# alv-around/mini-stark

Measured on AMD Instinct MI355X. Metric: stark_proofs_per_s, higher is better.
Workload: dtype u64; 1 GPU; Fibonacci AIR, Goldilocks, 2^20 trace rows, blowup 8, 20 security bits (w=3, c=6, rounds=23, ood_queries=1, fri_queries=2); a step = 8 independent proofs in flight per GPU

## Files before the change

### mini-stark_amd/csrc/ctx.hpp

```cpp
#pragma once
#include "../../include/ministark.h"

#include <cstdarg>
#include <cstdio>
#include <cstdlib>
#include <map>
#include <new>
#include <string>
#include <type_traits>
#include <vector>

#include "field.hpp"
#include "merkle.hpp"
#include "ntt.hpp"
#include "poly.hpp"

namespace msctx {

struct DevBuf {
  void* p = nullptr; size_t cap = 0;
  int ensure(size_t bytes) {
    if (bytes <= cap) return 0;
    if (p) msrt::free_dev(p);
    p = nullptr; cap = 0;
// ... 154 lines not shown
  msrt::HostFlag arm_flag() { if (!poll_sync || prof_on) return msrt::HostFlag{nullptr, 0}; seq_pending = ++seq_no; return msrt::HostFlag{host_seq(), seq_pending}; }
  void launched() { seq_armed = seq_pending; seq_pending = 0; }
  bool arm_next_eval = false;
  const unsigned long long* fwd_next_eval = nullptr;
  unsigned long long* host_aux2() const { return host_seq() + 1; }
  unsigned long long* validity_len_dev = nullptr; bool validity_len_host = false; size_t validity_ncoef = 0;
  DevBuf d_evdone;
  int ensure_evdone() { if (!d_evdone.p) { if (d_evdone.ensure(256)) return fail(MS_ERR_NOMEM, "length word"); CK(msrt::memset_dev(d_evdone.p, 0, 256, stream)); } return 0; }
  int sync_results() { const unsigned long long a = seq_armed; seq_armed = 0; return a ? msrt::sync_flag(stream, host_seq(), a) : msrt::sync(stream); }
  template <class K> int run_coop(int kid, unsigned gx, int threads, size_t lds, const typename K::Params& p, unsigned gy = 1) {
    launched();
    if (gx == 0 || gy == 0) return 0;
    if (!prof_on) return msrt::launch_coop<K>(stream, gx, gy, threads, lds, p);
    ProfRec r; r.kid = kid; r.sub = next_sub; r.bytes = next_bytes; r.part = part_depth > 0; next_bytes = 0; next_sub = 0;
    if (msrt::event_create(&r.a) || msrt::event_create(&r.b)) return 1;
    msrt::event_record(r.a, stream);
    int e = msrt::launch_coop<K>(stream, gx, gy, threads, lds, p);
    msrt::event_record(r.b, stream);
    prof_recs.push_back(r);
    return e;
  }
  template <class K> int run(int kid, unsigned gx, unsigned gy, int threads, size_t lds, const typename K::Params& p) {
    launched();
    if (gx == 0 || gy == 0) return 0;
    if (!prof_on) return msrt::launch<K>(stream, gx, gy, threads, lds, p);
    ProfRec r; r.kid = kid; r.sub = next_sub; r.bytes = next_bytes; r.part = part_depth > 0; next_bytes = 0; next_sub = 0;
    if (msrt::event_create(&r.a) || msrt::event_create(&r.b)) return 1;
    msrt::event_record(r.a, stream);
    int e = msrt::launch<K>(stream, gx, gy, threads, lds, p);
    msrt::event_record(r.b, stream);
    prof_recs.push_back(r);
    return e;
  }
  int profile_begin() override { prof_on = true; return 0; }
  int profile_end(char* out, size_t cap) override;

  struct Plan {
    int log_n = 0, log_r0 = 0, log_rho = 0, npass = 0, K[4] = {0, 0, 0, 0}, lo_bits = 0;
    int LC[4] = {msntt::TILE_LOG_C, msntt::TILE_LOG_C, msntt::TILE_LOG_C, msntt::TILE_LOG_C};
    bool v2[4] = {false, false, false, false};
    bool regp[4] = {false, false, false, false};
    DevBuf tw_lo, tw_hi, w_r[4], vtw, w0;
    T n_inv = 0;
  };
  std::map<int, Plan*> plans;
  DevBuf ntt_scratch;
  int ntt_kmax = 9;
  int ntt_v2 = 1, ntt_v2_regpass = 1;
  int ntt_fast = 1;

  int get_plan(int log_n, int log_pad, bool inverse, Plan** out);

  template <bool INV, int K, int TH>
  int launch_fast(const msntt::PassParams<F>& pp, size_t tiles, size_t batch);
  template <class KK> int launch_v2i(const msntt::PassParams<F>& pp, unsigned grid, int nsub, int mode, int k, int lc);
  template <bool INV, int K, int LC, int MODE>
  int launch_v2m(const msntt::PassParams<F>& pp, size_t tiles, size_t batch);
  int ntt_coop_wgs = 512, ntt_share = 1;
  unsigned coop_grid(size_t work_items, int per_cu = 2) const { const size_t g = (size_t)ntt_coop_wgs * per_cu / 2; return (unsigned)(work_items < g ? work_items : g); }
  template <bool INV, int K, int LC>
  int launch_v2(const msntt::PassParams<F>& pp, size_t tiles, size_t batch);
  template <bool INV, int LC>
  int launch_v2k(const msntt::PassParams<F>& pp, size_t tiles, size_t batch);
  template <bool INV, int K>
  int launch_reg(const msntt::PassParams<F>& pp, size_t batch);
  template <bool INV>
  int launch_pass(const msntt::PassParams<F>& pp, size_t tiles, size_t batch, bool v2 = false, bool regp = false);
// ... 52 lines not shown
  size_t lcount(const Round* r, size_t n) const { const size_t lo = (size_t)sh_rank * r->S; return n <= lo ? 0 : (n - lo < r->S ? n - lo : r->S); }
  size_t dist_chunk(size_t D) const {
    if (!sh_on || !shard_dist || !fri_blowup || !shardable(D / 2)) return 0;
    const size_t den = fri_blowup * (size_t)sh_world;
    if (D % den) return 0;
    const size_t S = D / den;
    return (S >= 2 && !(S & 1)) ? S : 0;
  }
  DevBuf d_carry, d_lq, d_pack, d_fullpoly;
  std::vector<Round*> rounds; size_t nrounds_done = 0, fri_rounds = 0, fri_blowup = 0;
  bool have_deep = false; XE cur_z; XE cur_B[2];
  DevBuf d_folded, d_sh, d_blob, d_tabs, d_targets, d_idx, d_deg, d_ovf;
  size_t blob_size = 0;

  int ensure_polys(size_t count);

  int init(int dev, u32 flags);
  ~Ctx() {
    for (auto& kv : plans) { kv.second->tw_lo.release(); kv.second->tw_hi.release(); kv.second->vtw.release(); kv.second->w0.release(); for (auto& b : kv.second->w_r) b.release(); delete kv.second; }
    drop_rccl();
    if (sdma_pending) msrt::Sdma::get().wait(sdma_sig, -1.0);
    else if (copy_pending) msrt::event_sync(ev_copy);
    if (up.pending) msrt::Sdma::get().wait(sdma_up_sig, -1.0);
    if (sdma_state == 1) { msrt::Sdma::get().signal_destroy(sdma_sig); msrt::Sdma::get().signal_destroy(sdma_up_sig); }
    for (msrt::Event* e : ev_hash) msrt::event_destroy(e);
    for (msrt::Event* e : ev_xchg) msrt::event_destroy(e);
    if (comm_stream) msrt::stream_destroy(comm_stream);
    if (side_stream) { msrt::sync(side_stream); msrt::stream_destroy(side_stream); }
    if (ev_side) msrt::event_destroy(ev_side);
    if (ev_blob) msrt::event_destroy(ev_blob);
    if (ev_copy) msrt::event_destroy(ev_copy);
    if (copy_stream) msrt::stream_destroy(copy_stream);
    for (Round* r : rounds) { r->poly.release(); r->cw.release(); r->nodes.release(); delete r; }
    DevBuf* bufs[] = {&ntt_scratch, &d_trace[0], &d_trace[1], &d_polys, &d_coef, &d_lde, &d_trace_nodes, &d_lde_nodes, &d_io, &d_partials, &d_small, &d_folded, &d_sh, &d_blob, &d_tabs, &d_targets, &d_idx, &d_deg, &d_ovf, &d_zero, &d_lin, &d_cubic, &d_carry, &d_lq, &d_pack, &d_fullpoly, &d_evdone};
    for (DevBuf* b : bufs) b->release();
    if (pinned) msrt::free_host(pinned);
    if (h_tabs) msrt::free_host(h_tabs);
    if (own_stream) msrt::stream_destroy(own_stream);
  }
  int ext_degree() const override { return E; }
  void bind_device() const override { msrt::set_device(device); }
  int set_stream(void* s) override { stream = s ? reinterpret_cast<msrt::Stream*>(s) : own_stream; zero_used = zero_cap; return 0; }
  int synchronize() override { CK(msrt::sync(stream)); return 0; }

  static unsigned grid1(size_t n, int threads) { return (unsigned)((n + threads - 1) / threads); }

  int upload_narrow(const u64* host, size_t n, T* dst);
  int transpose_in(const u64* src, T* dst, size_t rows, size_t cols, T rinv, int mont, u32* bad);
  int download_widen(const T* src, size_t n, size_t limb_stride, u32 e, u64* host);
  static bool canonical(const u64* v, size_t n) { for (size_t i = 0; i < n; i++) if (v[i] >= F::P) return false; return true; }

  int trace_commit(const u64* trace, bool on_device, size_t N_, size_t w_, size_t lpn, u8* root) override;
  int interpolate() override;
  int polys_lincomb(const u64* s, const int* idx, int k) override;
  int polys_append(const u64* coeffs, size_t n) override;
  int polys_count() const override { return npolys; }
  int poly_read(int i, u64* out) override;

  int lincomb_into(const T* base, size_t stride, size_t n, const u64* sc, const int* idx, int k, int self_index, T* dst);
  int lincomb_linear_columns(T* base, size_t stride, size_t n);
  int lde_compute(size_t blowup_, u64 shift);
  int lde_virtual = -1; bool lde_cols_virtual = false; size_t lde_col_stride = 0, lde_col_len = 0;
  DevBuf d_lin;
  int finish_linear_columns(size_t stride, size_t n);
  const msmerkle::LinColSpec* lde_lin() const { return lde_cols_virtual ? d_lin.as<msmerkle::LinColSpec>() : nullptr; }
  int coset_eval(const T* coef, size_t coef_bstride, size_t ncoef, int log_D, T shift, size_t g, T* dst, size_t dst_bstride, size_t batch);
  int lde_compute_sharded(size_t blowup_, u64 shift);
// ... 114 lines not shown
```

### mini-stark_amd/csrc/merkle.hpp

```cpp
#pragma once
#include "field.hpp"

namespace msmerkle {

constexpr int THREADS = 256;
constexpr int OVF_WORDS = 2;
constexpr int OVF_LISTS = 256;
constexpr int PAD_GRID_Y = 4;
struct alignas(16) uint4_t { u32 x, y, z, w; };

MS_HD u32 rotr32(u32 x, int n) {
#if defined(__HIP_DEVICE_COMPILE__)
  return __builtin_amdgcn_alignbit(x, x, n);
#else
  return (x >> n) | (x << (32 - n));
#endif
}
MS_HD u32 bswap32(u32 x) { return __builtin_bswap32(x); }
MS_HD u32 ch3(u32 e, u32 f, u32 g) {
#if defined(__HIP_DEVICE_COMPILE__) && __has_builtin(__builtin_amdgcn_bitop3_b32)
  return __builtin_amdgcn_bitop3_b32(e, f, g, 0xCA);
#else
  return g ^ (e & (f ^ g));
#endif
// ... 49 lines not shown
    u32 a = st[0], b = st[1], c = st[2], d = st[3], e = st[4], f = st[5], g = st[6], h = st[7];
#pragma unroll
    for (int i = 0; i < 64; i++) {
      if (i >= 16) {
        u32 w15 = w[(i + 1) & 15], w2 = w[(i + 14) & 15];
        u32 s0 = xor3(rotr32(w15, 7), rotr32(w15, 18), w15 >> 3);
        u32 s1 = xor3(rotr32(w2, 17), rotr32(w2, 19), w2 >> 10);
        w[i & 15] = w[i & 15] + s0 + w[(i + 9) & 15] + s1;
      }
      u32 S1 = xor3(rotr32(e, 6), rotr32(e, 11), rotr32(e, 25));
      u32 ch = ch3(e, f, g);
      u32 t1 = h + S1 + ch + SHA_K[i] + w[i & 15];
      u32 S0 = xor3(rotr32(a, 2), rotr32(a, 13), rotr32(a, 22));
      u32 mj = maj3(a, b, c);
      u32 t2 = S0 + mj;
      h = g; g = f; f = e; e = d + t1; d = c; c = b; b = a; a = t1 + t2;
    }
    st[0] += a; st[1] += b; st[2] += c; st[3] += d; st[4] += e; st[5] += f; st[6] += g; st[7] += h;
  }
  template <u32 MSG_BITS> MS_HD void compress_pad_block() {
    u32 a = st[0], b = st[1], c = st[2], d = st[3], e = st[4], f = st[5], g = st[6], h = st[7];
#pragma unroll
    for (int i = 0; i < 64; i++) {
      u32 S1 = xor3(rotr32(e, 6), rotr32(e, 11), rotr32(e, 25));
      u32 ch = ch3(e, f, g);
      u32 t1 = h + S1 + ch + PadBlock<MSG_BITS>::T.kw[i];
      u32 S0 = xor3(rotr32(a, 2), rotr32(a, 13), rotr32(a, 22));
      u32 mj = maj3(a, b, c);
      u32 t2 = S0 + mj;
      h = g; g = f; f = e; e = d + t1; d = c; c = b; b = a; a = t1 + t2;
    }
    st[0] += a; st[1] += b; st[2] += c; st[3] += d; st[4] += e; st[5] += f; st[6] += g; st[7] += h;
  }
};

#ifndef MS_SUBTREE_PAIR_LEVELS
#define MS_SUBTREE_PAIR_LEVELS 1
#endif
struct Sha256Pair {
  u32 M, R1, R2, R3, Sa, Sb, Sc;
  bool a_lane;
  u32 cv[4];
  static MS_HD bool is_a_lane(int lane) { return (lane >> 2) & 1; }
  static MS_HD int node_in_group(int lane) { return is_a_lane(lane) ? 3 - (lane & 3) : (lane & 3); }
  MS_DEV void init(int lane) {
    a_lane = is_a_lane(lane);
    M = a_lane ? ~0u : 0u;
    R1 = a_lane ? 2 : 6; R2 = a_lane ? 13 : 11; R3 = a_lane ? 22 : 25;
    Sa = a_lane ? 17 : 7; Sb = a_lane ? 19 : 18; Sc = a_lane ? 10 : 3;
  }
  MS_DEV void reset() {
    cv[0] = a_lane ? 0x6a09e667u : 0x510e527fu; cv[1] = a_lane ? 0xbb67ae85u : 0x9b05688cu; cv[2] = a_lane ? 0x3c6ef372u : 0x1f83d9abu; cv[3] = a_lane ? 0xa54ff53au : 0x5be0cd19u;
  }
  MS_DEV void round(u32& x, u32& y, u32& z, u32& v, u32 kw) const {
    const u32 S = xor3(msrt::rotr_var(x, R1), msrt::rotr_var(x, R2), msrt::rotr_var(x, R3));
    const u32 xp = ms_bitop3<0x78>(x, z, M);
    const u32 F = ch3(xp, y, z);
    const u32 s = S + F;
    const u32 t = s + v + kw;
    const u32 n = msrt::pair_exchange_add(a_lane, v, t, s);
    v = z; z = y; y = x; x = n;
  }
  MS_DEV void compress(u32 (&w)[16]) {
    u32 x = cv[0], y = cv[1], z = cv[2], v = cv[3];
#pragma unroll
    for (int i = 0; i < 64; i++) {
      if (i >= 16) {
// ... 98 lines not shown
      for (int i = 0; i < 16; i++) w[i] = buf[i * NT];
#pragma unroll
      for (int i = 0; i < 16; i++) w[i] = (done + i < valid_end) ? w[i] : 0u;
      if (pending == 16) { w[14] = 0; w[15] = msg_bytes * 8u; }
      h.compress(w);
      done += 16;
      return pending == 32 ? DEFER : DONE;
    } else {
      const bool last = limit - done == 16;
      if (limit - 16 >= valid_end && last) return DEFER;
      u32 w[16];
      const u32* blk = buf + (done - fbase) * NT;
#pragma unroll
      for (int i = 0; i < 16; i++) w[i] = (done + i < valid_end) ? blk[i * NT] : 0u;
      if (last) { w[14] = 0; w[15] = msg_bytes * 8u; }
      h.compress(w);
      done += 16;
      if (limit == done) return DONE;
      return (limit - 16 >= valid_end && limit - done == 16) ? DEFER : MORE;
    }
  }
};

MS_HD u32 bcd4(u32 c) {
  const u32 q = (c * 5243u) >> 19;
  const u32 t = c + q * 65436u;
  const u32 tens = ((t * 103u) >> 10) & 0x000F000Fu;
  const u32 ones = t - tens * 10u;
  return (tens << 8) + ones;
}
MS_HD u32 pack4(u32 c) { return bcd4(c) + 0x30303030u; }
MS_HD u32 clz32(u32 x) { return (u32)__builtin_clz(x); }

MS_HD void dec_chunks(const GL&, u64 v, u32 (&c)[5]) {
  const u32 vh = (u32)(v >> 32);
  u32 q1 = (u32)(((u64)vh * 1934281311u) >> 32) >> 20;
  u64 r = v - (u64)q1 * 10000000000000000ULL;
  if (r >= 10000000000000000ULL) { r -= 10000000000000000ULL; q1++; }
  const u32 x = (u32)(r >> 22);
  u32 q2 = (u32)(((u64)x * 180143985u) >> 32);
  u32 r2 = (u32)r - q2 * 100000000u;
  if (r2 >= 100000000u) { r2 -= 100000000u; q2++; }
  c[0] = q1;
  c[1] = q2 / 10000u; c[2] = q2 - c[1] * 10000u;
  c[3] = r2 / 10000u; c[4] = r2 - c[3] * 10000u;
}
MS_HD void dec_chunks(const BB&, u64 v, u32 (&c)[3]) {
  const u32 x = (u32)v;
  c[0] = x / 100000000u; const u32 r = x - c[0] * 100000000u;
  c[1] = r / 10000u; c[2] = r - c[1] * 10000u;
}

template <class F, class S> MS_HD void put_dec(S& s, typename F::T v_, int zero_as_empty) {
  const u64 v = F::to_u64(v_);
  constexpr int NCH = (F::MAX_DIGITS + 3) / 4;
  u32 c[NCH];
  dec_chunks(F(), v, c);
  if (c[0] != 0) {
    u32 W[NCH];
    const u32 b0 = bcd4(c[0]);
    const u32 lead = clz32(b0) >> 3;
    W[0] = b0 + 0x30303030u;
#pragma unroll
    for (int j = 1; j < NCH; j++) W[j] = pack4(c[j]);
    const u32 sel = drop_sel(lead);
    u32 X[NCH];
#pragma unroll
    for (int j = 0; j + 1 < NCH; j++) X[j] = drop_bytes(W[j], W[j + 1], lead, sel);
    X[NCH - 1] = drop_bytes(W[NCH - 1], 0u, lead, sel);
    s.template append_words<NCH>(X, 4u * NCH - lead, W[NCH - 1]);
    return;
  }
  if (v == 0) { if (!zero_as_empty) s.append_small(0x30000000u, 1); return; }
  u32 lead = 0; bool found = false;
#pragma unroll
  for (int j = 0; j < NCH; j++) {
    const u32 z = c[j] == 0 ? 4u : (c[j] < 10u ? 3u : (c[j] < 100u ? 2u : (c[j] < 1000u ? 1u : 0u)));
    if (!found) lead += z;
    found = found || (c[j] != 0);
  }
  for (int j = 1; j < NCH; j++) {
    const int k = 4 * (j + 1) - (int)lead;
    if (k >= 4) s.append_small(pack4(c[j]), 4);
    else if (k > 0) s.append_small(pack4(c[j]) << (8 * (4 - k)), (u32)k);
  }
}
template <int E> struct Affix;
template <> struct Affix<1> {
  static constexpr int MAX_BYTES = 0;
  template <class S> static MS_HD void before(S&, u32) {}
  template <class S> static MS_HD void after(S&, u32) {}
};
template <class S> MS_HD void put_open(S& s) { const u32 W[4] = {0x51756164u, 0x45787446u, 0x69656c64u, 0x28000000u}; s.template append_words<4>(W, 13, 0x656c6428u); }
template <class S> MS_HD void put_plus(S& s) { s.append_small(0x202b2000u, 3); }
template <class S> MS_HD void put_close(S& s) { const u32 W[2] = {0x202a2075u, 0x29000000u}; s.template append_words<2>(W, 5, 0x2a207529u); }
template <> struct Affix<2> {
  static constexpr int MAX_BYTES = 13;
  template <class S> static MS_HD void before(S& s, u32 k) { if (k == 0) put_open(s); else put_plus(s); }
  template <class S> static MS_HD void after(S& s, u32 k) { if (k == 1) put_close(s); }
};
template <> struct Affix<4> {
  static constexpr int MAX_BYTES = 26;
  template <class S> static MS_HD void before(S& s, u32 k) {
    if (k == 0) {
      const u32 W[7] = {0x51756164u, 0x45787446u, 0x69656c64u, 0x28517561u, 0x64457874u, 0x4669656cu, 0x64280000u};
      s.template append_words<7>(W, 26, 0x656c6428u);
// ... 8 lines not shown
      const u32 W[3] = {0x202a2075u, 0x29202a20u, 0x75290000u};
      s.template append_words<3>(W, 10, 0x2a207529u);
    }
  }
};

constexpr int LIN_MAXT = 4;
struct LinColSpec { u32 n ; u32 src[LIN_MAXT]; u64 s[LIN_MAXT]; };
struct Sha256Kernels;
template <class F, int E, bool LAZY = false, class DG = Sha256Kernels> struct LeafHashKernel {
  typedef typename F::T T;
  static constexpr int THREADS = msmerkle::THREADS;
  struct Params {
    const T* base; size_t col_stride, row_stride, limb_stride;
    u32 width, lpn; int zero_as_empty;
    size_t ngroups;
    u32* nodes;
    u32* ovf_count; u32* ovf; u32 ovf_cap;
    size_t g_first; u32 run_len, run_stride;
    const LinColSpec* lin;
    size_t out_g0;
  };
  static constexpr int MAX_BYTES = F::MAX_DIGITS + Affix<E>::MAX_BYTES;
  static constexpr int MAXW = (3 + MAX_BYTES + 3) / 4 + 1;
  static constexpr int NWORDS = (LAZY ? 32 : 16) + MAXW + 1 + DG::EXTRA_WORDS;
  typedef typename DG::template Stream<NWORDS, THREADS, MAXW, LAZY> Stream;
  static MS_HD int nphases(const Params&) { return 1; }
  static MS_HD size_t lds_bytes() { return (size_t)NWORDS * THREADS * sizeof(u32); }
  static MS_DEV void phase(int, const Params& p, int bx, int, int tid, int nthreads, unsigned char* lds) {
    size_t g = (size_t)bx * nthreads + tid;
    if (g >= p.ngroups) return;
    if (p.run_len) g = p.g_first + (g / p.run_len) * (size_t)p.run_stride + g % p.run_len;
    Stream s; s.init(reinterpret_cast<u32*>(lds), tid);
    size_t f = g * p.lpn;
    size_t row = f / p.width; u32 col = (u32)(f - row * p.width);
    const u32 nlimbs = p.lpn * (u32)E;
    u32 msg_bytes = 0;
    bool deferred = false;
    for (u32 j = 0; LAZY || j <= nlimbs; j++) {
      if (j < nlimbs) {
        const u32 k = j & (u32)(E - 1);
        const T* rowp = p.base + row * p.row_stride + (size_t)k * p.limb_stride;
        T v;
        if (p.lin && p.lin[col].n) {
          const LinColSpec& lc = p.lin[col];
          v = 0;
          for (u32 t = 0; t < lc.n; t++) {
            const T x = rowp[(size_t)lc.src[t] * p.col_stride];
            if (lc.s[t] == 1) v = F::add(v, x);
            else if (lc.s[t] == F::P - 1) v = F::sub(v, x);
            else v = F::add(v, F::mul(x, F::from_u64(lc.s[t])));
          }
        } else v = rowp[(size_t)col * p.col_stride];
        Affix<E>::before(s, k);
        put_dec<F>(s, v, p.zero_as_empty);
        Affix<E>::after(s, k);
        if (k == (u32)(E - 1) && ++col == p.width) { col = 0; row++; }
      } else if (j == nlimbs) {
        msg_bytes = s.end_message();
      }
      const int st = s.drain(j >= nlimbs, msg_bytes);
      if constexpr (LAZY) { if (j >= nlimbs && st != Stream::MORE) { deferred = st == Stream::DEFER; break; } }
      else deferred = st == Stream::DEFER;
    }
    if constexpr (!DG::DEFERS) { s.store_digest(p.nodes + (g - p.out_g0) * 8); }
    else {
      if (deferred && !p.ovf) {
        u32 w[16];
#pragma unroll
        for (int i = 0; i < 15; i++) w[i] = 0;
        w[15] = msg_bytes * 8u;
        s.h.compress(w);
        deferred = false;
      }
      const u32 list = (u32)bx % (u32)OVF_LISTS;
      const u32 slot = msrt::wave_alloc_slot(p.ovf_count + list, deferred);
      const size_t go = g - p.out_g0;
      if (deferred) {
        u32* e = p.ovf + ((size_t)list * p.ovf_cap + slot) * OVF_WORDS;
        e[0] = (u32)go; e[1] = msg_bytes * 8u;
        u32* st = p.nodes + go * 8;
#pragma unroll
        for (int i = 0; i < 8; i++) st[i] = s.h.st[i];
        return;
      }
      s.store_digest(p.nodes + go * 8);
    }
  }
};
struct PadOnlyBlockKernel {
  static constexpr int THREADS = msmerkle::THREADS;
  struct Params { const u32* ovf_count; const u32* ovf; u32 ovf_cap; u32* nodes; };
  static MS_HD int nphases(const Params&) { return 1; }
  static MS_DEV void phase(int, const Params& p, int bx, int by, int tid, int nthreads, unsigned char*) {
    const u32 n = p.ovf_count[bx];
    const u32 stride = (u32)nthreads * PAD_GRID_Y;
    for (u32 t = (u32)by * nthreads + tid; t < n; t += stride) {
      const u32* e = p.ovf + ((size_t)bx * p.ovf_cap + t) * OVF_WORDS;
      Sha256 h;
      const u32* st = p.nodes + (size_t)e[0] * 8;
#pragma unroll
      for (int i = 0; i < 8; i++) h.st[i] = st[i];
      u32 w[16];
#pragma unroll
      for (int i = 0; i < 15; i++) w[i] = 0;
      w[15] = e[1];
      h.compress(w);
      uint4_t* out = reinterpret_cast<uint4_t*>(p.nodes + (size_t)e[0] * 8);
      uint4_t o0, o1;
      o0.x = bswap32(h.st[0]); o0.y = bswap32(h.st[1]); o0.z = bswap32(h.st[2]); o0.w = bswap32(h.st[3]);
      o1.x = bswap32(h.st[4]); o1.y = bswap32(h.st[5]); o1.z = bswap32(h.st[6]); o1.w = bswap32(h.st[7]);
      out[0] = o0; out[1] = o1;
    }
  }
};

struct InnerHashParams { u32* nodes; size_t child_off, nchildren; u32 ic; u32 nlevels; u32* host_root;
                         unsigned long long* aux_src; unsigned long long* aux_dst;
                         msrt::HostFlag flag;  };
template <int IC> struct InnerHashKernelT {
  static constexpr int THREADS = msmerkle::THREADS;
  typedef InnerHashParams Params;
  static MS_HD int nphases(const Params& p) { return (int)p.nlevels; }
  static MS_DEV void phase(int ph, const Params& p, int bx, int, int tid, int nthreads, unsigned char*) {
    const u32 ic = IC ? (u32)IC : p.ic;
    size_t child_off = p.child_off, nchildren = p.nchildren;
    for (int l = 0; l < ph; l++) { child_off += nchildren; nchildren /= ic; }
    const size_t nparents = nchildren / ic;
    const size_t stride = (p.nlevels > 1) ? (size_t)nthreads : 0;
    for (size_t g = (size_t)bx * nthreads + tid; g < nparents; g += stride) {
      const u32* ch = p.nodes + (child_off + g * ic) * 8;
      Sha256 h; h.init();
      u32 w[16];
      for (u32 b = 0; b < ic / 2; b++) {
        const uint4_t* c4 = reinterpret_cast<const uint4_t*>(ch + b * 16);
#pragma unroll
        for (int q = 0; q < 4; q++) {
          const uint4_t v = c4[q];
          w[4 * q] = bswap32(v.x); w[4 * q + 1] = bswap32(v.y); w[4 * q + 2] = bswap32(v.z); w[4 * q + 3] = bswap32(v.w);
        }
        h.compress(w);
      }
      if constexpr (IC > 0) h.template compress_pad_block<(u32)IC * 256u>();
      else {
        w[0] = 0x80000000u;
// ... 276 lines not shown
```

### mini-stark_amd/csrc/merkle_tree.cpp

```cpp
#include "ctx.hpp"
#include "blake2s.hpp"
#include "blake3.hpp"

namespace msctx {

template <class F>
int Ctx<F>::tree_shape(size_t leaf_num, size_t lpn, size_t ic, TreeShape* ts) {
  if (lpn == 0 || ic < 2 || !is_pow2(ic)) return fail(MS_ERR_SHAPE, "merkle: bad leafs_per_node / inner_children");
  const size_t node_num = leaf_num / lpn;
  long lg = log_two_k(node_num, ic);
  if (lg < 0) return fail(MS_ERR_SHAPE, lg == -1 ? "number if not a power of 2" : "number if not a power of base");
  if (leaf_num % lpn != 0) return fail(MS_ERR_SHAPE, "merkle: leaf_num % leafs_per_node != 0");
  if (lg >= 64 || node_num == 0) return fail(MS_ERR_SHAPE, "Tree is not full!");
  ts->leaf_num = leaf_num; ts->lpn = lpn; ts->ic = ic; ts->levels = (size_t)lg + 1;
  size_t total = 0, m = node_num;
  for (;;) { total += m; if (m == 1) break; m /= ic; }
  ts->nodes = total; ts->local_nodes = total; ts->Mloc = 0; ts->sharded = false;
  return 0;
}

template <class F> template <int EL>
int Ctx<F>::leaf_hash(const T* base, size_t col_stride, size_t row_stride, size_t limb_stride, u32 width, size_t lpn, size_t ngroups, u32* out,
              size_t g_first, u32 run_len, u32 run_stride, const msmerkle::LinColSpec* lin, size_t out_g0) {
  if (ngroups >> 32) return fail(MS_ERR_SHAPE, "more than 2^32 leaf groups");
// ... 14 lines not shown
      const size_t bound = lpn * EL * (size_t)msmerkle::LeafHashKernel<F, EL, false, msmerkle::Blake3Kernels>::MAX_BYTES;
      if (lpn > msmerkle::B3_MAX_BYTES || bound > msmerkle::B3_MAX_BYTES)
        return fail(MS_ERR_ARG, "BLAKE3: a leaf group's message may exceed 16384 bytes (leafs_per_node x limbs x longest decimal): not supported by the BLAKE3 kernels");
      if (bound > msmerkle::B3_CHUNK_BYTES) {
        if (lazy) return launch(msmerkle::LeafHashKernel<F, EL, true, msmerkle::Blake3MultiKernels>());
        return launch(msmerkle::LeafHashKernel<F, EL, false, msmerkle::Blake3MultiKernels>());
      }
      if (lazy) return launch(msmerkle::LeafHashKernel<F, EL, true, msmerkle::Blake3Kernels>());
      return launch(msmerkle::LeafHashKernel<F, EL, false, msmerkle::Blake3Kernels>());
    }
    if (lazy) return launch(msmerkle::LeafHashKernel<F, EL, true, msmerkle::Blake2sKernels>());
    return launch(msmerkle::LeafHashKernel<F, EL, false, msmerkle::Blake2sKernels>());
  }
  const size_t nwg = grid1(ngroups, msmerkle::THREADS), lists = msmerkle::OVF_LISTS;
  const size_t cap = ((nwg + lists - 1) / lists) * msmerkle::THREADS;
  if (d_ovf.ensure(lists * cap * msmerkle::OVF_WORDS * 4)) return fail(MS_ERR_NOMEM, "deferred-block lists");
  void* counters;
  RQ(zero_alloc(lists * 4, &counters));
  typename msmerkle::LeafHashKernel<F, EL>::Params lp;
  lp.base = base; lp.col_stride = col_stride; lp.row_stride = row_stride; lp.limb_stride = limb_stride;
  lp.width = width; lp.lpn = (u32)lpn; lp.zero_as_empty = zae; lp.ngroups = ngroups; lp.nodes = out;
  lp.ovf_count = reinterpret_cast<u32*>(counters); lp.ovf = d_ovf.as<u32>(); lp.ovf_cap = (u32)cap;
  lp.g_first = g_first; lp.run_len = run_len; lp.run_stride = run_stride; lp.lin = lin; lp.out_g0 = out_g0;
  next_bytes = (double)ngroups * (lpn * EL * sizeof(T) + 32);
  if (lpn * EL >= (size_t)leaf_lazy_min) {
    typedef msmerkle::LeafHashKernel<F, EL, true> LK;
    typename LK::Params ll;
    ll.base = lp.base; ll.col_stride = lp.col_stride; ll.row_stride = lp.row_stride; ll.limb_stride = lp.limb_stride; ll.width = lp.width; ll.lpn = lp.lpn;
    ll.zero_as_empty = lp.zero_as_empty; ll.ngroups = lp.ngroups; ll.nodes = lp.nodes; ll.ovf_count = lp.ovf_count; ll.ovf = lp.ovf; ll.ovf_cap = lp.ovf_cap;
    ll.g_first = g_first; ll.run_len = run_len; ll.run_stride = run_stride; ll.lin = lin; ll.out_g0 = out_g0;
    CK(run<LK>(K_LEAF_HASH, grid1(ngroups, msmerkle::THREADS), 1, msmerkle::THREADS, LK::lds_bytes(), ll));
  } else
  CK(run<msmerkle::LeafHashKernel<F, EL>>(K_LEAF_HASH, grid1(ngroups, msmerkle::THREADS), 1, msmerkle::THREADS, msmerkle::LeafHashKernel<F, EL>::lds_bytes(), lp));
  msmerkle::PadOnlyBlockKernel::Params pp{lp.ovf_count, lp.ovf, (u32)cap, out};
  const size_t used = nwg < lists ? nwg : lists, per_list = grid1(cap, msmerkle::THREADS);
  CK(run<msmerkle::PadOnlyBlockKernel>(K_LEAF_HASH, (unsigned)used, (unsigned)(per_list < (size_t)msmerkle::PAD_GRID_Y ? per_list : (size_t)msmerkle::PAD_GRID_Y), msmerkle::THREADS, 0, pp));
  return 0;
}

template <class F> template <int EL>
int Ctx<F>::tree_build(const T* base, size_t col_stride, size_t row_stride, size_t limb_stride, u32 width, const TreeShape& ts, DevBuf& nodes, const msmerkle::LinColSpec* lin) {
  if (nodes.ensure(ts.nodes * 32)) return fail(MS_ERR_NOMEM, "merkle nodes");
  const size_t ngroups = ts.leaf_num / ts.lpn;
  RQ((leaf_hash<EL>(base, col_stride, row_stride, limb_stride, width, ts.lpn, ngroups, nodes.as<u32>(), 0, 0, 0, lin)));
  RQ(inner_levels(nodes.as<u32>(), ngroups, ts.ic));
  return 0;
}

template <class F>
int Ctx<F>::inner_launch(unsigned grid, const msmerkle::InnerHashParams& ip) {
  if (digest == MS_DIGEST_BLAKE3) {
    if (ip.ic > msmerkle::B3InnerHashMultiKernel::MAX_IC) return fail(MS_ERR_ARG, "BLAKE3: inner nodes of more than 512 children (16384 bytes) are not supported by the BLAKE3 kernels");
    if (ip.ic == 2) CK(run<msmerkle::B3InnerHashKernel2>(K_INNER_HASH, grid, 1, msmerkle::THREADS, 0, ip));
    else if (ip.ic <= msmerkle::B3InnerHashKernel::MAX_IC) CK(run<msmerkle::B3InnerHashKernel>(K_INNER_HASH, grid, 1, msmerkle::THREADS, 0, ip));
    else CK(run<msmerkle::B3InnerHashMultiKernel>(K_INNER_HASH, grid, 1, msmerkle::THREADS, msmerkle::B3InnerHashMultiKernel::lds_bytes(), ip));
  } else if (digest == MS_DIGEST_BLAKE2S256) {
    if (ip.ic == 2) CK(run<msmerkle::B2InnerHashKernel2>(K_INNER_HASH, grid, 1, msmerkle::THREADS, 0, ip));
    else CK(run<msmerkle::B2InnerHashKernel>(K_INNER_HASH, grid, 1, msmerkle::THREADS, 0, ip));
  } else {
    if (ip.ic == 2) CK(run<msmerkle::InnerHashKernel2>(K_INNER_HASH, grid, 1, msmerkle::THREADS, 0, ip));
    else CK(run<msmerkle::InnerHashKernel>(K_INNER_HASH, grid, 1, msmerkle::THREADS, 0, ip));
  }
  return 0;
}

template <class F>
int Ctx<F>::inner_levels(u32* nodes, size_t nchildren, size_t ic, bool final_levels, u8* rec_out) {
  size_t child_off = 0;
  if (final_levels) root_on_host = false;
// ... 169 lines not shown
```

### mini-stark_amd/csrc/session.cpp

```cpp
#include "ctx.hpp"

namespace msctx {

template <class F>
int Ctx<F>::profile_end(char* out, size_t cap) {
  static const char* names[K_COUNT] = {"ntt_pass", "scale_pow", "leaf_hash", "inner_hash", "transpose_in", "io_copy", "lincomb", "mix", "eval", "eval_reduce",
                                       "fold", "suffix_horner", "degree", "find_first", "merkle_path", "query_points", "fri_tail"};
  msrt::sync(stream);
  double ms[K_COUNT] = {0}, by[K_COUNT] = {0}, ms_part = 0, ms_repl = 0, repl_by[K_COUNT] = {0}; unsigned long long cnt[K_COUNT] = {0};
  std::map<int, double> sub_ms, sub_by; std::map<int, unsigned long long> sub_cnt;
  for (auto& r : prof_recs) {
    float t = 0.f; msrt::event_elapsed_ms(&t, r.a, r.b);
    ms[r.kid] += t; by[r.kid] += r.bytes; cnt[r.kid]++;
    if (r.part) ms_part += t; else { ms_repl += t; repl_by[r.kid] += t; }
    if (r.kid == K_NTT_PASS) { sub_ms[r.sub] += t; sub_by[r.sub] += r.bytes; sub_cnt[r.sub]++; }
    msrt::event_destroy(r.a); msrt::event_destroy(r.b);
  }
  prof_recs.clear(); prof_on = false;
  std::string j = "{";
  for (int k = 0; k < K_COUNT; k++) {
    char buf[256];
    snprintf(buf, sizeof buf, "%s\"%s\": {\"launches\": %llu, \"ms\": %.6f, \"alg_bytes\": %.0f}", k ? ", " : "", names[k], cnt[k], ms[k], by[k]);
    j += buf;
  }
  j += ", \"ntt_pass_variants\": {";
  bool first = true;
  for (auto& kv : sub_ms) {
    const int sub = kv.first; char buf[420];
    const char* name = ntt_names[(size_t)sub < ntt_names.size() ? sub : 0].c_str();
    snprintf(buf, sizeof buf, "%s\"%s\": {\"launches\": %llu, \"ms\": %.6f, \"alg_bytes\": %.0f}", first ? "" : ", ", name, sub_cnt[sub], kv.second, sub_by[sub]);
    j += buf; first = false;
  }
  j += "}";
  { char buf[200]; snprintf(buf, sizeof buf, ", \"shard\": {\"world\": %d, \"partitioned_ms\": %.6f, \"replicated_ms\": %.6f, \"replicated_by_kernel\": {", sh_world, ms_part, ms_repl); j += buf;
    bool first_k = true;
    for (int k = 0; k < K_COUNT; k++) if (repl_by[k] > 0) { snprintf(buf, sizeof buf, "%s\"%s\": %.4f", first_k ? "" : ", ", names[k], repl_by[k]); j += buf; first_k = false; }
    j += "}}}"; }
  if (out && cap) { size_t n = j.size() < cap - 1 ? j.size() : cap - 1; memcpy(out, j.data(), n); out[n] = 0; }
  return 0;
}

template <class F>
int Ctx<F>::tabs_host(size_t bytes, u8** out) {
  CK(msrt::sync(stream));
  if (bytes > h_tabs_cap) {
    if (h_tabs) msrt::free_host(h_tabs);
    h_tabs = nullptr; h_tabs_cap = 0;
    const size_t want = bytes + bytes / 4 + 4096;
    if (msrt::malloc_host(&h_tabs, want)) { h_tabs = nullptr; return fail(MS_ERR_NOMEM, "page-locked table staging"); }
    h_tabs_cap = want;
  }
  *out = reinterpret_cast<u8*>(h_tabs);
  return 0;
}

// ... 42 lines not shown
  if (const char* e = getenv("MS_NTT_SHARE")) ntt_share = atoi(e);
  if (const char* e = getenv("MS_NTT_COOP_WGS")) { int v = atoi(e); if (v >= 8 && v <= 65536) ntt_coop_wgs = v & ~7; }
  if (const char* e = getenv("MS_LDE_LINEAR")) lde_linear = atoi(e);
  if (const char* e = getenv("MS_LAZY_LINCOMB")) lazy_lin = atoi(e);
  if (const char* e = getenv("MS_LDE_MULTI")) lde_multi = atoi(e);
  if (const char* e = getenv("MS_LDE_VIRTUAL")) lde_virtual = atoi(e);
  if (const char* e = getenv("MS_FRI_POINTWISE")) fri_pointwise = atoi(e);
  if (const char* e = getenv("MS_FOLD_SMALL_MAX")) fold_small_max = (size_t)atol(e);
  if (const char* e = getenv("MS_FRI_TAIL_MAX")) fri_tail_max = (size_t)atol(e);
  if (const char* e = getenv("MS_FRI_OVERLAP")) fri_overlap = atoi(e);
  if (const char* e = getenv("MS_SYNC_POLL")) poll_sync = atoi(e);
  if (const char* e = getenv("MS_EVAL_SMALL_MAX")) eval_small_max = (size_t)atol(e);
  if (const char* e = getenv("MS_TREE_SUBTREE_PARENTS")) subtree_parents = (size_t)atol(e);
  if (const char* e = getenv("MS_UPLOAD")) upload_sdma = !strcmp(e, "hip") ? 0 : 1;
  if (const char* e = getenv("MS_SDMA_TIMEOUT_S")) { const double v = atof(e); if (v > 0) sdma_timeout_s = v; }
  if (const char* e = getenv("MS_READBACK")) readback_sdma = !strcmp(e, "hip") ? 0 : (!strcmp(e, "sdma-async") ? 1 : 2);
  if (const char* e = getenv("MS_LEAF_LAZY_MIN")) leaf_lazy_min = atoi(e);
  if (const char* e = getenv("MS_TREE_TOP")) { int v = atoi(e); if (v >= 1 && v <= 65536) tree_top_parents = v; }
  if (const char* e = getenv("MS_SHARD_MIN_LEAVES")) { long v = atol(e); if (v >= 1) shard_min_leaves = (size_t)v; }
  if (const char* e = getenv("MS_SHARD_DIST")) shard_dist = atoi(e);
  if (const char* e = getenv("MS_SHARD_WORLD1")) allow_w1 = atoi(e);
  if (const char* e = getenv("MS_SHARD_STUB")) shard_stub = atoi(e);
  if (const char* e = getenv("MS_SHARD_GATHER_CHUNK")) { long v = atol(e); if (v >= 64) shard_gather_chunk = (size_t)v & ~(size_t)63; }
  if (const char* e = getenv("MS_SHARD_SLICES")) { int v = atoi(e); if (v >= 1 && v <= 64) { shard_slices = v; shard_slices_set = true; } }
  if (const char* e = getenv("MS_SHARD_SLICE_MIN")) { long v = atol(e); if (v >= 1) shard_slice_min = (size_t)v; }
  if (const char* e = getenv("MS_RCCL_MAX_PIECE")) { long long v = atoll(e); if (v >= 64 && v <= ((long long)1 << 30)) rccl_max_piece = (size_t)v & ~(size_t)63; }
  CK(msrt::set_device(dev));
  CK(msrt::stream_create(&own_stream));
  stream = own_stream;
  pinned_cap = 1 << 16;
  CK(msrt::malloc_host_coherent(&pinned, pinned_cap + 64));
  *host_seq() = 0;
  if (d_small.ensure(4096)) return fail(MS_ERR_NOMEM, "small");
  return 0;
}

template <class F>
int Ctx<F>::upload_narrow(const u64* host, size_t n, T* dst) {
  if (d_io.ensure(n * 8)) return fail(MS_ERR_NOMEM, "io staging");
  CK(msrt::h2d(d_io.p, host, n * 8, stream));
  typename mspoly::NarrowKernel<F>::Params p{d_io.as<u64>(), dst, n};
  CK(run<mspoly::NarrowKernel<F>>(K_IO, grid1(n, mspoly::THREADS), 1, mspoly::THREADS, 0, p));
  return 0;
}

template <class F>
int Ctx<F>::download_widen(const T* src, size_t n, size_t limb_stride, u32 e, u64* host) {
  if (n == 0) return 0;
  if (d_io.ensure(n * e * 8)) return fail(MS_ERR_NOMEM, "io staging");
  typename mspoly::WidenKernel<F>::Params p{src, d_io.as<u64>(), n, limb_stride, e};
  CK(run<mspoly::WidenKernel<F>>(K_IO, grid1(n * e, mspoly::THREADS), 1, mspoly::THREADS, 0, p));
  CK(msrt::d2h(host, d_io.p, n * e * 8, stream));
  CK(msrt::sync(stream));
  return 0;
}

template <class F>
int Ctx<F>::transpose_in(const u64* src, T* dst, size_t rows, size_t cols, T rinv, int mont, u32* bad) {
  typename mspoly::TransposeInKernel<F>::Params tp{src, dst, rows, cols, rows, rinv, mont, bad};
  if (cols >= 16 && rows >= 64) {
    typedef mspoly::TransposeInTiledKernel<F> TK;
    CK(run<TK>(K_TRANSPOSE, (unsigned)(rows / TK::TILE), (unsigned)((cols + TK::TILE - 1) / TK::TILE), TK::THREADS, TK::lds_bytes(), tp));
  } else
  CK(run<mspoly::TransposeInKernel<F>>(K_TRANSPOSE, grid1(rows * cols, mspoly::THREADS), 1, mspoly::THREADS, 0, tp));
  return 0;
}
// ... 121 lines not shown
```

Measured before the change: 277.0 proofs/s.

## Use precomputed SHA-256 pad-only message schedule table in leaf hashing

Result: no change. 278.4 proofs/s (median of 2 runs) (+0.5%).

```diff
diff --git a/mini-stark_amd/csrc/ctx.hpp b/mini-stark_amd/csrc/ctx.hpp
--- a/mini-stark_amd/csrc/ctx.hpp
+++ b/mini-stark_amd/csrc/ctx.hpp
@@ -210,7 +210,14 @@
     prof_recs.push_back(r);
     return e;
   }
-  int profile_begin() override { prof_on = true; return 0; }
+  DevBuf d_padkw, d_padstat; u32 pad_table_rows = msmerkle::PAD_TABLE_ROWS_DEFAULT;
+  int profile_begin() override {
+    if (digest == MS_DIGEST_SHA256) {
+      if (d_padstat.ensure(8)) return fail(MS_ERR_NOMEM, "pad-only block counters");
+      CK(msrt::memset_dev(d_padstat.p, 0, 8, stream));
+    }
+    prof_on = true; return 0;
+  }
   int profile_end(char* out, size_t cap) override;
 
   struct Plan {
@@ -329,7 +336,7 @@
     if (ev_copy) msrt::event_destroy(ev_copy);
     if (copy_stream) msrt::stream_destroy(copy_stream);
     for (Round* r : rounds) { r->poly.release(); r->cw.release(); r->nodes.release(); delete r; }
-    DevBuf* bufs[] = {&ntt_scratch, &d_trace[0], &d_trace[1], &d_polys, &d_coef, &d_lde, &d_trace_nodes, &d_lde_nodes, &d_io, &d_partials, &d_small, &d_folded, &d_sh, &d_blob, &d_tabs, &d_targets, &d_idx, &d_deg, &d_ovf, &d_zero, &d_lin, &d_cubic, &d_carry, &d_lq, &d_pack, &d_fullpoly, &d_evdone};
+    DevBuf* bufs[] = {&ntt_scratch, &d_trace[0], &d_trace[1], &d_polys, &d_coef, &d_lde, &d_trace_nodes, &d_lde_nodes, &d_io, &d_partials, &d_small, &d_folded, &d_sh, &d_blob, &d_tabs, &d_targets, &d_idx, &d_deg, &d_ovf, &d_zero, &d_lin, &d_cubic, &d_carry, &d_lq, &d_pack, &d_fullpoly, &d_evdone, &d_padkw, &d_padstat};
     for (DevBuf* b : bufs) b->release();
     if (pinned) msrt::free_host(pinned);
     if (h_tabs) msrt::free_host(h_tabs);
diff --git a/mini-stark_amd/csrc/merkle.hpp b/mini-stark_amd/csrc/merkle.hpp
--- a/mini-stark_amd/csrc/merkle.hpp
+++ b/mini-stark_amd/csrc/merkle.hpp
@@ -105,7 +105,39 @@
     }
     st[0] += a; st[1] += b; st[2] += c; st[3] += d; st[4] += e; st[5] += f; st[6] += g; st[7] += h;
   }
-};
+  MS_HD void compress_kw(const u32* kw) {
+    u32 a = st[0], b = st[1], c = st[2], d = st[3], e = st[4], f = st[5], g = st[6], h = st[7];
+#pragma unroll
+    for (int i = 0; i < 64; i++) {
+      u32 S1 = xor3(rotr32(e, 6), rotr32(e, 11), rotr32(e, 25));
+      u32 ch = ch3(e, f, g);
+      u32 t1 = h + S1 + ch + kw[i];
+      u32 S0 = xor3(rotr32(a, 2), rotr32(a, 13), rotr32(a, 22));
+      u32 mj = maj3(a, b, c);
+      u32 t2 = S0 + mj;
+      h = g; g = f; f = e; e = d + t1; d = c; c = b; b = a; a = t1 + t2;
+    }
+    st[0] += a; st[1] += b; st[2] += c; st[3] += d; st[4] += e; st[5] += f; st[6] += g; st[7] += h;
+  }
+};
+constexpr u32 PAD_ROW_WORDS = 64, PAD_TABLE_ROWS_DEFAULT = 512, PAD_ROW_NONE = 0xFFFFFFFEu;
+MS_HD u32 pad_row_of_bits(u32 msg_bits) {
+  const u32 len = msg_bits >> 3;
+  return ((msg_bits & 7u) == 0 && (len & 63u) >= 56u) ? (((len >> 6) << 3) | (len & 7u)) : PAD_ROW_NONE;
+}
+constexpr u32 pad_row_bits(u32 row) { return (((row >> 3) << 6) + 56u + (row & 7u)) * 8u; }
+constexpr PadBlockKW make_pad_only_kw(u32 msg_bits) {
+  PadBlockKW r{};
+  u32 w[64] = {};
+  w[15] = msg_bits;
+  for (int i = 16; i < 64; i++) {
+    const u32 s0 = c_rotr(w[i - 15], 7) ^ c_rotr(w[i - 15], 18) ^ (w[i - 15] >> 3);
+    const u32 s1 = c_rotr(w[i - 2], 17) ^ c_rotr(w[i - 2], 19) ^ (w[i - 2] >> 10);
+    w[i] = w[i - 16] + s0 + w[i - 7] + s1;
+  }
+  for (int i = 0; i < 64; i++) r.kw[i] = SHA_K[i] + w[i];
+  return r;
+}
 
 #ifndef MS_SUBTREE_PAIR_LEVELS
 #define MS_SUBTREE_PAIR_LEVELS 1
@@ -270,7 +302,7 @@
 MS_HD u32 pack4(u32 c) { return bcd4(c) + 0x30303030u; }
 MS_HD u32 clz32(u32 x) { return (u32)__builtin_clz(x); }
 
-MS_HD void dec_chunks(const GL&, u64 v, u32 (&c)[5]) {
+MS_HD void dec_split(const GL&, u64 v, u32& q1_, u32 (&half)[2]) {
   const u32 vh = (u32)(v >> 32);
   u32 q1 = (u32)(((u64)vh * 1934281311u) >> 32) >> 20;
   u64 r = v - (u64)q1 * 10000000000000000ULL;
@@ -279,28 +311,27 @@
   u32 q2 = (u32)(((u64)x * 180143985u) >> 32);
   u32 r2 = (u32)r - q2 * 100000000u;
   if (r2 >= 100000000u) { r2 -= 100000000u; q2++; }
-  c[0] = q1;
-  c[1] = q2 / 10000u; c[2] = q2 - c[1] * 10000u;
-  c[3] = r2 / 10000u; c[4] = r2 - c[3] * 10000u;
-}
-MS_HD void dec_chunks(const BB&, u64 v, u32 (&c)[3]) {
+  q1_ = q1; half[0] = q2; half[1] = r2;
+}
+MS_HD void dec_split(const BB&, u64 v, u32& q1, u32 (&half)[1]) {
   const u32 x = (u32)v;
-  c[0] = x / 100000000u; const u32 r = x - c[0] * 100000000u;
-  c[1] = r / 10000u; c[2] = r - c[1] * 10000u;
+  q1 = x / 100000000u; half[0] = x - q1 * 100000000u;
 }
 
 template <class F, class S> MS_HD void put_dec(S& s, typename F::T v_, int zero_as_empty) {
   const u64 v = F::to_u64(v_);
+  if (v == 0) { if (!zero_as_empty) s.append_small(0x30000000u, 1); return; }
   constexpr int NCH = (F::MAX_DIGITS + 3) / 4;
-  u32 c[NCH];
-  dec_chunks(F(), v, c);
-  if (c[0] != 0) {
+  constexpr int NH = (NCH - 1) / 2;
+  u32 q1, half[NH];
+  dec_split(F(), v, q1, half);
+  if (q1 != 0) {
     u32 W[NCH];
-    const u32 b0 = bcd4(c[0]);
+    const u32 b0 = bcd4(q1);
     const u32 lead = clz32(b0) >> 3;
     W[0] = b0 + 0x30303030u;
 #pragma unroll
-    for (int j = 1; j < NCH; j++) W[j] = pack4(c[j]);
+    for (int j = 0; j < NH; j++) { const u32 hi = half[j] / 10000u; W[1 + 2 * j] = pack4(hi); W[2 + 2 * j] = pack4(half[j] - hi * 10000u); }
     const u32 sel = drop_sel(lead);
     u32 X[NCH];
 #pragma unroll
@@ -309,7 +340,10 @@
     s.template append_words<NCH>(X, 4u * NCH - lead, W[NCH - 1]);
     return;
   }
-  if (v == 0) { if (!zero_as_empty) s.append_small(0x30000000u, 1); return; }
+  u32 c[NCH];
+  c[0] = 0;
+#pragma unroll
+  for (int j = 0; j < NH; j++) { c[1 + 2 * j] = half[j] / 10000u; c[2 + 2 * j] = half[j] - c[1 + 2 * j] * 10000u; }
   u32 lead = 0; bool found = false;
 #pragma unroll
   for (int j = 0; j < NCH; j++) {
@@ -384,8 +418,10 @@
     if (g >= p.ngroups) return;
     if (p.run_len) g = p.g_first + (g / p.run_len) * (size_t)p.run_stride + g % p.run_len;
     Stream s; s.init(reinterpret_cast<u32*>(lds), tid);
-    size_t f = g * p.lpn;
-    size_t row = f / p.width; u32 col = (u32)(f - row * p.width);
+    size_t row; u32 col;
+    if (p.width == 1) { row = g * p.lpn; col = 0; }
+    else if (p.width == p.lpn) { row = g; col = 0; }
+    else { const size_t f = g * p.lpn; row = f / p.width; col = (u32)(f - row * p.width); }
     const u32 nlimbs = p.lpn * (u32)E;
     u32 msg_bytes = 0;
     bool deferred = false;
@@ -442,27 +478,60 @@
 };
 struct PadOnlyBlockKernel {
   static constexpr int THREADS = msmerkle::THREADS;
-  struct Params { const u32* ovf_count; const u32* ovf; u32 ovf_cap; u32* nodes; };
-  static MS_HD int nphases(const Params&) { return 1; }
-  static MS_DEV void phase(int, const Params& p, int bx, int by, int tid, int nthreads, unsigned char*) {
+  static constexpr u32 LDS_ROWS = 8;
+  struct Params { const u32* ovf_count; const u32* ovf; u32 ovf_cap; u32* nodes;
+                  const u32* kw_table; u32 table_rows;
+                  u32* stat; };
+  static MS_HD size_t lds_bytes() { return (size_t)LDS_ROWS * PAD_ROW_WORDS * sizeof(u32); }
+  static MS_DEV void run(const Params& p, int bx, int by, int, int tid, unsigned char* lds) {
+    u32* const rows = reinterpret_cast<u32*>(lds);
+    const u32* const list = p.ovf + (size_t)bx * p.ovf_cap * OVF_WORDS;
     const u32 n = p.ovf_count[bx];
-    const u32 stride = (u32)nthreads * PAD_GRID_Y;
-    for (u32 t = (u32)by * nthreads + tid; t < n; t += stride) {
-      const u32* e = p.ovf + ((size_t)bx * p.ovf_cap + t) * OVF_WORDS;
-      Sha256 h;
-      const u32* st = p.nodes + (size_t)e[0] * 8;
+    const u32 first_bits = list[1];
+    const u32 stride = (u32)THREADS * PAD_GRID_Y;
+    u32 t = (u32)by * THREADS + (u32)tid;
+    if ((u32)by * THREADS >= n) return;
+    u32 e0 = 0, e1 = 0;
+    Sha256 h;
+    auto fetch = [&]() {
+      e0 = list[(size_t)t * OVF_WORDS]; e1 = list[(size_t)t * OVF_WORDS + 1];
+      const u32* st = p.nodes + (size_t)e0 * 8;
 #pragma unroll
       for (int i = 0; i < 8; i++) h.st[i] = st[i];
-      u32 w[16];
-#pragma unroll
-      for (int i = 0; i < 15; i++) w[i] = 0;
-      w[15] = e[1];
-      h.compress(w);
-      uint4_t* out = reinterpret_cast<uint4_t*>(p.nodes + (size_t)e[0] * 8);
+    };
+    if (t < n) fetch();
+    u32 lo = PAD_ROW_NONE;
+    if (p.kw_table) {
+      const u32 r0 = pad_row_of_bits(first_bits);
+      if (r0 != PAD_ROW_NONE && (r0 | (LDS_ROWS - 1)) < p.table_rows) {
+        lo = r0 & ~(LDS_ROWS - 1);
+        for (u32 i = (u32)tid; i < LDS_ROWS * PAD_ROW_WORDS; i += (u32)THREADS) rows[i] = p.kw_table[(size_t)lo * PAD_ROW_WORDS + i];
+      }
+      msrt::wg_barrier_global();
+    }
+    u32 from_table = 0, computed = 0;
+    while (t < n) {
+      const u32 r = pad_row_of_bits(e1) - lo;
+      if (lo != PAD_ROW_NONE && r < LDS_ROWS) { h.compress_kw(rows + r * PAD_ROW_WORDS); from_table++; }
+      else {
+        u32 w[16];
+#pragma unroll
+        for (int i = 0; i < 15; i++) w[i] = 0;
+        w[15] = e1;
+        h.compress(w);
+        computed++;
+      }
+      uint4_t* out = reinterpret_cast<uint4_t*>(p.nodes + (size_t)e0 * 8);
       uint4_t o0, o1;
       o0.x = bswap32(h.st[0]); o0.y = bswap32(h.st[1]); o0.z = bswap32(h.st[2]); o0.w = bswap32(h.st[3]);
       o1.x = bswap32(h.st[4]); o1.y = bswap32(h.st[5]); o1.z = bswap32(h.st[6]); o1.w = bswap32(h.st[7]);
       out[0] = o0; out[1] = o1;
+      t += stride;
+      if (t < n) fetch();
+    }
+    if (p.stat) {
+      if (from_table) msrt::atomic_add_u32(p.stat, from_table);
+      if (computed) msrt::atomic_add_u32(p.stat + 1, computed);
     }
   }
 };
diff --git a/mini-stark_amd/csrc/merkle_tree.cpp b/mini-stark_amd/csrc/merkle_tree.cpp
--- a/mini-stark_amd/csrc/merkle_tree.cpp
+++ b/mini-stark_amd/csrc/merkle_tree.cpp
@@ -70,9 +70,10 @@
     CK(run<LK>(K_LEAF_HASH, grid1(ngroups, msmerkle::THREADS), 1, msmerkle::THREADS, LK::lds_bytes(), ll));
   } else
   CK(run<msmerkle::LeafHashKernel<F, EL>>(K_LEAF_HASH, grid1(ngroups, msmerkle::THREADS), 1, msmerkle::THREADS, msmerkle::LeafHashKernel<F, EL>::lds_bytes(), lp));
-  msmerkle::PadOnlyBlockKernel::Params pp{lp.ovf_count, lp.ovf, (u32)cap, out};
+  typedef msmerkle::PadOnlyBlockKernel PK;
+  PK::Params pp{lp.ovf_count, lp.ovf, (u32)cap, out, d_padkw.as<u32>(), d_padkw.p ? pad_table_rows : 0, prof_on ? d_padstat.as<u32>() : nullptr};
   const size_t used = nwg < lists ? nwg : lists, per_list = grid1(cap, msmerkle::THREADS);
-  CK(run<msmerkle::PadOnlyBlockKernel>(K_LEAF_HASH, (unsigned)used, (unsigned)(per_list < (size_t)msmerkle::PAD_GRID_Y ? per_list : (size_t)msmerkle::PAD_GRID_Y), msmerkle::THREADS, 0, pp));
+  CK(run_coop<PK>(K_LEAF_HASH, (unsigned)used, PK::THREADS, PK::lds_bytes(), pp, (unsigned)(per_list < (size_t)msmerkle::PAD_GRID_Y ? per_list : (size_t)msmerkle::PAD_GRID_Y)));
   return 0;
 }
 
diff --git a/mini-stark_amd/csrc/session.cpp b/mini-stark_amd/csrc/session.cpp
--- a/mini-stark_amd/csrc/session.cpp
+++ b/mini-stark_amd/csrc/session.cpp
@@ -17,10 +17,13 @@
     msrt::event_destroy(r.a); msrt::event_destroy(r.b);
   }
   prof_recs.clear(); prof_on = false;
+  u32 pad_stat[2] = {0, 0};
+  if (d_padstat.p) { CK(msrt::d2h(pad_stat, d_padstat.p, sizeof pad_stat, stream)); CK(msrt::sync(stream)); }
   std::string j = "{";
   for (int k = 0; k < K_COUNT; k++) {
-    char buf[256];
-    snprintf(buf, sizeof buf, "%s\"%s\": {\"launches\": %llu, \"ms\": %.6f, \"alg_bytes\": %.0f}", k ? ", " : "", names[k], cnt[k], ms[k], by[k]);
+    char buf[320];
+    if (k == K_LEAF_HASH) snprintf(buf, sizeof buf, "%s\"%s\": {\"launches\": %llu, \"ms\": %.6f, \"alg_bytes\": %.0f, \"pad_only_table_blocks\": %u, \"pad_only_computed_blocks\": %u}", k ? ", " : "", names[k], cnt[k], ms[k], by[k], pad_stat[0], pad_stat[1]);
+    else snprintf(buf, sizeof buf, "%s\"%s\": {\"launches\": %llu, \"ms\": %.6f, \"alg_bytes\": %.0f}", k ? ", " : "", names[k], cnt[k], ms[k], by[k]);
     j += buf;
   }
   j += ", \"ntt_pass_variants\": {";
@@ -129,6 +132,17 @@
   CK(msrt::malloc_host_coherent(&pinned, pinned_cap + 64));
   *host_seq() = 0;
   if (d_small.ensure(4096)) return fail(MS_ERR_NOMEM, "small");
+  if (const char* e = getenv("MS_PAD_TABLE_ROWS")) { long v = atol(e); if (v >= 0 && v <= 4096) pad_table_rows = (u32)v; }
+  if (digest == MS_DIGEST_SHA256 && pad_table_rows) {
+    std::vector<u32> kw((size_t)pad_table_rows * msmerkle::PAD_ROW_WORDS);
+    for (u32 r = 0; r < pad_table_rows; r++) {
+      const msmerkle::PadBlockKW row = msmerkle::make_pad_only_kw(msmerkle::pad_row_bits(r));
+      memcpy(&kw[(size_t)r * msmerkle::PAD_ROW_WORDS], row.kw, sizeof row.kw);
+    }
+    if (d_padkw.ensure(kw.size() * 4)) return fail(MS_ERR_NOMEM, "pad-only table");
+    CK(msrt::h2d(d_padkw.p, kw.data(), kw.size() * 4, stream));
+    CK(msrt::sync(stream));
+  }
   return 0;
 }
 
```
